# actionml/universal-recommender

Hardware: NVIDIA H100
Metric: CCO train events/sec to indicator model (higher is better)
Workload: dtype int32+f64

## Files before the change

universal_recommender_b200/csrc/cco_api.cu:

```cuda
#include <cuda_runtime.h>
#include <dlfcn.h>
#include <stdarg.h>
#include <stdio.h>
#include <stdlib.h>
#include <string.h>

#include <algorithm>
#include <cmath>
#include <functional>
#include <cub/cub.cuh>
#include <nvtx3/nvToolsExt.h>
#include <condition_variable>
#include <mutex>
#include <string>
#include <thread>
#include <unordered_map>
#include <vector>

#include "../../include/cco_b200.h"
#include "cco_kernels.cuh"
#include "cco_sampler.cuh"
#include "cco_format.cuh"
#include "cco_strings.cuh"
#include "cco_json.cuh"
// ... 637 lines not shown
  }
  CK(cudaEventRecord(stage_ev[2], s));
  if (W > 1) {
    g_nccl.GroupStart();
    for (int i = 0; i < n_mats; ++i) {
      if (!gathered[i]) continue;
      int rc = g_nccl.AllGather(gathered[i] + (size_t)r * cap[i], gathered[i], (size_t)cap[i], kNcclInt32, c->comm, s);
      if (rc != 0) { g_nccl.GroupEnd(); return nccl_check(rc, "ncclAllGather(column blocks)"); }
    }
    CKR(nccl_check(g_nccl.GroupEnd(), "ncclGroupEnd(column blocks)"));
    for (int i = 0; i < n_mats; ++i) {
      if (!gathered[i]) continue;
      dim3 grid((unsigned)std::max(1, std::min(c->sm_count * 8 / W, 1024)), (unsigned)W);
      k_pack_blocks<<<grid, 256, 0, s>>>(W, S, U, cap[i], dm[i].rp, gathered[i], dm[i].col);
      c->launches++;
      ar.release(gathered[i]);
    }
  }
  CK(cudaEventRecord(stage_ev[3], s));
  CK(cudaGetLastError());
  return CCO_OK;
}


struct BinCfg {
  int group;
  int slots;
  int cap;
  int cbuf;
  int caux, keep_max, final_max;
  bool dense;
  bool bitmap;
  int bm_words;
  size_t region;
  size_t smem;
  int ctas_per_sm;
};

static int next_pow2(int x) {
  int p = 1;
  while (p < x) p <<= 1;
  return p;
}

template <int GROUP>
static int launch_rows_t(cco_ctx *c, const RowArgs &a, BinCfg &cfg, cudaStream_t st) {
  constexpr int CTA = GROUP == 32 ? 64 : GROUP;
  int occ = 1;
  void (*kern)(const RowArgs) = cfg.dense ? k_rows<GROUP, true> : k_rows<GROUP, false>;
  if constexpr (GROUP == 512 || GROUP == 256)
    if (cfg.bitmap) kern = k_rows<GROUP, false, true>;
  CK(cudaFuncSetAttribute(kern, cudaFuncAttributeMaxDynamicSharedMemorySize, (int)cfg.smem));
  CK(cudaOccupancyMaxActiveBlocksPerMultiprocessor(&occ, kern, CTA, cfg.smem));
  kern<<<c->sm_count * std::max(occ, 1) * 4, CTA, cfg.smem, st>>>(a);
  cfg.ctas_per_sm = occ;
  c->launches++;
  CK(cudaGetLastError());
  return CCO_OK;
}
static int launch_rows(cco_ctx *c, const RowArgs &a, BinCfg &cfg, cudaStream_t st) {
  switch (cfg.group) {
    case 1024: return launch_rows_t<1024>(c, a, cfg, st);
    case 512: return launch_rows_t<512>(c, a, cfg, st);
    case 256: return launch_rows_t<256>(c, a, cfg, st);
    case 128: return launch_rows_t<128>(c, a, cfg, st);
    case 32: return launch_rows_t<32>(c, a, cfg, st);
  }
  return set_error(CCO_E_INVALID_ARG, "internal: bad bin config");
}

static BinCfg make_cfg(cco_ctx *c, int group, int want_slots, int top_k, int n_cols_b) {
  BinCfg f;
  const int groups = group == 32 ? 2 : 1;
  f.group = group;
  f.final_max = next_pow2(top_k);
  f.cbuf = next_pow2(top_k + std::max(group, 128) + (group == 32 ? 64 : 0));
  if (group == 32 && top_k + 32 <= 96) f.cbuf = 128;
  f.keep_max = std::max(f.final_max, (f.cbuf - group) / 2);
  f.caux = group == 32 ? 0 : f.keep_max;
  size_t fixed = (size_t)(f.cbuf + f.caux) * 16 + 2 * 256 + 512 + 1024 + (size_t)(group / 32) * 256;
  size_t avail = (c->smem_optin - 1024) / groups;
  int max_slots = (int)((avail - fixed) / 4) & ~1023;
  f.slots = std::min(want_slots, max_slots);
  f.cap = f.slots / 2;
  f.dense = n_cols_b <= f.slots;
  f.bitmap = false;
  f.bm_words = 0;
  f.region = (fixed + (size_t)f.slots * 4 + 15) & ~(size_t)15;
  f.smem = f.region * groups;
  f.ctas_per_sm = 1;
  return f;
}

static bool use_bitmap(BinCfg &f, uint32_t max_w, int top_k, int n_cols_b) {
  if (f.dense || (f.group != 512 && f.group != 256)) return false;
  const long long seg = 32LL * (f.group / 32);
  const long long rep = (std::max<long long>(max_w, 64) + seg - 1) / seg * seg;
  const long long bm = ((long long)n_cols_b + 31) / 32;
  if (rep + bm + top_k > f.slots) return false;
  f.bitmap = true;
  f.slots = (int)rep;
  f.bm_words = (int)bm;
  return true;
}

static double llr_error_bound(long long n_users) {
  const double n = (double)n_users;
  return n > 1.0 ? std::ldexp(n * std::log(n), -47) : 0.0;
}
static bool cut_exact(long long n_users, int32_t max_marg_a, int32_t max_marg_b) {
  const double n = (double)n_users, r = (double)max_marg_a, c = (double)max_marg_b;
  if (r <= 0.0 || c <= 0.0) return true;
  double g = 2.0 / std::min(r * c, 0.5 * n);
  const double d = n - c - r + 1.0;
  if (d > 0.0) g = std::max(g, 2.0 * (1.0 / c - (r - 1.0) / d));
  return g > 2.0 * llr_error_bound(n_users);
}

struct IndicatorState {
  int mail_group = -1;
// ... 43 lines not shown
  CKR(ar.alloc(&rows_sorted, n_items_a + 1));
  CK(cudaMemsetAsync(work64 + n_items_a, 0, 8, ss));
  k_row_work<<<grid_for((long long)n_items_a * kSG, 256, c->sm_count), 256, 0, ss>>>(n_items_a, at_ptr, at_users, B.rp,
                                                                                  row_work, work64, ids, nullptr);
  c->launches++;
  CKR(exclusive_sum(c, ar, (const long long *)work64, work_prefix, (long long)n_items_a + 1, ss));
  if (world > 1) {
    CKR(ar.alloc(&d_pb, world + 1));
    k_partition_rows<<<1, ((world + 1 + 31) / 32) * 32, 0, ss>>>(work_prefix, n_items_a, world, d_pb);
    c->launches++;
  }
  k_mask_work<<<grid_for(n_items_a, 256, c->sm_count), 256, 0, ss>>>(n_items_a, row_work, d_pb, rank, masked);
  c->launches++;
  if (n_items_a > 0) {
    void *tmp;
    CKR(ar.alloc((char **)&tmp, sort_tb));
    CK(cub::DeviceRadixSort::SortPairsDescending(tmp, sort_tb, masked, sorted_work, ids, rows_sorted, n_items_a, 0, 32, ss));
    ar.release(tmp);
  }
  const int k_eff = emit_all ? 1 : prm.top_k;
  const bool warp_ok = k_eff + 32 <= 256;
  struct BinSpec { int group, slots; uint32_t max_w; };
  std::vector<BinSpec> spec = {{1024, 1 << 20, 0xffffffffu}, {1024, 1 << 20, 0xffffffffu}, {512, 16384, 8192u}, {256, 8192, 4096u}};
  if (warp_ok) {
    spec.push_back({128, 4096, 2048u});
    spec.push_back({32, 2048, 1024u});
    spec.push_back({32, 1024, 512u});
    spec.push_back({32, 512, 256u});
  } else {
    spec.push_back({128, 4096, 2048u});
  }
  const int kBins = (int)spec.size();
  std::vector<BinCfg> cfgs(kBins);
  for (int b = 0; b < kBins; ++b) cfgs[b] = make_cfg(c, spec[b].group, spec[b].slots, k_eff, n_cols_b);
  BinCfg &cfgL = cfgs[1];
  int key_bits = 1;
  while (((1LL << key_bits) - 1) <= (long long)n_cols_b) ++key_bits;
  int count_bits = 32 - key_bits;
  const long long k11_max = std::min<long long>(max_marg_a, max_marg_b);
  if (count_bits < 1 || k11_max >= (1LL << count_bits))
    return set_error(CCO_E_UNSUPPORTED,
                     "co-occurrence counts up to %lld over %d columns do not fit the packed 32-bit accumulator word "
                     "(key %d bits + count %d bits): lower maxItemsPerUser/maxEventsPerEventType for this event type "
                     "(\"Limits\" in include/cco_b200.h)", k11_max, n_cols_b, key_bits, count_bits);
  std::vector<uint32_t> h_thr(kBins);
  for (int b = 0; b < kBins; ++b) {
    const BinCfg &f = cfgs[std::min(b + 1, kBins - 1)];
    uint32_t lim = b + 1 < kBins ? spec[b + 1].max_w : 0u;
    if (b + 1 < kBins && !f.dense) lim = std::min<uint32_t>(lim, (uint32_t)f.cap);
    h_thr[b] = lim;
    if (b > 0) h_thr[b] = std::min(h_thr[b], h_thr[b - 1]);
  }
  const bool bitmap_ok = !emit_all && cut_exact(n_users, max_marg_a, max_marg_b) &&
                         2ull * (unsigned long long)std::max(max_marg_a, 0) * (unsigned long long)std::max(max_marg_b, 0) <
                             (unsigned long long)n_users;
  for (int b = 1; b < kBins && bitmap_ok; ++b) use_bitmap(cfgs[b], h_thr[b - 1], k_eff, n_cols_b);
  int32_t *d_bounds;
  CKR(ar.alloc(&d_bounds, kBins + 3));
  BinThresholds bt;
  memset(&bt, 0, sizeof bt);
  for (int b = 0; b < kBins; ++b) bt.t[b] = h_thr[b];
  k_bin_bounds<<<1, 32, 0, ss>>>(n_items_a, sorted_work, kBins, bt, d_bounds);
  c->launches++;
  int32_t *key_of_col, *first_key_of_cb, *order_id0, *order_id1;
  uint32_t *order_cb0, *order_cb1;
  const int32_t n_order = std::max<int32_t>(n_cols_b, 1);
  CKR(ar.alloc(&key_of_col, n_order));
// ... 66 lines not shown
  a.self = self ? 1 : 0;
  a.top_k = k_eff;
  a.has_min_llr = prm.has_min_llr;
  a.min_llr = prm.min_llr;
  a.cut_ok = cut_exact(n_users, max_marg_a, max_marg_b) ? 1 : 0;
  a.llr_eps2 = 2.0 * llr_error_bound(n_users);
  a.flags = flags;
  a.count_bits = count_bits;
  a.out_stride = stride;
  a.out_col = o_col;
  a.out_llr = o_llr;
  a.out_cnt = o_cnt;
  a.out_len = o_len;
  a.stat_distinct = d_distinct;
  a.stat_evaluated = d_distinct + 1;
  a.err_flag = d_err;
  a.emit_all = emit_all ? 1 : 0;
  if (ev_begin) CK(cudaEventRecord(ev_begin, s));
  if (n_items_a > 0) {
    CK(cudaEventRecord(c->bin_ev[8], s));
    for (int b = 0; b < kBins; ++b) {
      if (b == 0 && cfgL.dense) continue;
      RowArgs ab = a;
      ab.bin = b;
      ab.slots = cfgs[b].slots;
      ab.cap = cfgs[b].cap;
      ab.tsize_x16 = 32;
      ab.cbuf = cfgs[b].cbuf;
      ab.caux = cfgs[b].caux;
      ab.keep_max = cfgs[b].keep_max;
      ab.final_max = cfgs[b].final_max;
      ab.group_smem_bytes = (int32_t)cfgs[b].region;
      ab.bm_words = cfgs[b].bm_words;
      CK(cudaStreamWaitEvent(c->bin_stream[b], c->bin_ev[8], 0));
      CKR(launch_rows(c, ab, cfgs[b], c->bin_stream[b]));
      CK(cudaEventRecord(c->bin_ev[b], c->bin_stream[b]));
      CK(cudaStreamWaitEvent(s, c->bin_ev[b], 0));
    }
  }
  if (ev_end) CK(cudaEventRecord(ev_end, s));
  long long *len64, *rec_d;
  CKR(ar.alloc(&len64, n_items_a + 1));
  CKR(ar.alloc(&st->out_ptr, n_items_a + 1));
  CKR(ar.alloc(&rec_d, 8));
  k_len_to_i64<<<grid_for((long long)n_items_a + 1, 256, c->sm_count), 256, 0, s>>>(n_items_a, o_len, d_pb, rank, len64);
  c->launches++;
  CKR(exclusive_sum(c, ar, len64, st->out_ptr, (long long)n_items_a + 1));
  CKR(ar.alloc(&st->p_col, cells));
  if (!(flags & CCO_FLAG_RESULT_NO_COUNT) || emit_all) CKR(ar.alloc(&st->p_cnt, cells));
  if (!emit_all && !(flags & CCO_FLAG_RESULT_NO_LLR)) CKR(ar.alloc(&st->p_llr, cells));
  if (n_items_a > 0) {
    k_compact_rows<<<grid_for((long long)n_items_a * 32, 256, c->sm_count), 256, 0, s>>>(n_items_a, stride, st->out_ptr, o_col, o_llr,
                                                                                      o_cnt, st->p_col, st->p_llr, st->p_cnt);
    c->launches++;
  }
  k_indicator_record<<<1, 32, 0, s>>>(n_items_a, d_pb, rank, st->out_ptr, work_prefix, d_distinct, d_err, rec_d);
  c->launches++;
  CKR(mail_fetch(c, st->rec, rec_d, sizeof(long long) * 7));
  CKR(mail_close(c, &st->mail_group));
  if (!st->packed) CK(cudaEventCreateWithFlags(&st->packed, cudaEventDisableTiming));
  CK(cudaEventRecord(st->packed, s));
  CK(cudaGetLastError());
  for (void *p : {(void *)o_col, (void *)o_cnt, (void *)o_llr, (void *)len64})
    if (p) ar.release(p);
  return CCO_OK;
}
// ... 4743 lines not shown
  CK(cudaMemcpyAsync(score, d_score, sizeof(double) * (size_t)n_items, cudaMemcpyDeviceToHost, s));
  CK(cudaMemcpyAsync(present, d_present, (size_t)n_items, cudaMemcpyDeviceToHost, s));
  CK(cudaStreamSynchronize(s));
  CK(cudaGetLastError());
  return CCO_OK;
}

void cco_free(void *p) { free(p); }

int cco_debug_llr(cco_ctx_t *c, int64_t n, const int64_t *k11, const int64_t *k12, const int64_t *k21, const int64_t *k22,
                  uint32_t flags, double *out) {
  if (!c || n < 0 || (n > 0 && (!k11 || !k12 || !k21 || !k22 || !out))) return set_error(CCO_E_INVALID_ARG, "bad argument");
  if (n == 0) return CCO_OK;
  for (int64_t i = 0; i < n; ++i)
    if (k11[i] < 0 || k12[i] < 0 || k21[i] < 0 || k22[i] < 0)
      return set_error(CCO_E_INVALID_ARG, "negative count at %lld (Preconditions.checkArgument in LogLikelihood)", (long long)i);
  CK(cudaSetDevice(c->device));
  Arena ar(c->stream);
  long long *d[4];
  double *dout;
  const int64_t *h[4] = {k11, k12, k21, k22};
  for (int j = 0; j < 4; ++j) {
    CKR(ar.alloc(&d[j], n));
    CK(cudaMemcpyAsync(d[j], h[j], sizeof(int64_t) * (size_t)n, cudaMemcpyHostToDevice, c->stream));
  }
  CKR(ar.alloc(&dout, n));
  k_debug_llr<<<(unsigned)((n + 255) / 256), 256, 0, c->stream>>>(n, d[0], d[1], d[2], d[3], flags, dout);
  CK(cudaMemcpyAsync(out, dout, sizeof(double) * (size_t)n, cudaMemcpyDeviceToHost, c->stream));
  CK(cudaStreamSynchronize(c->stream));
  CK(cudaGetLastError());
  return CCO_OK;
}

int cco_debug_rank_text(cco_ctx_t *c, int64_t n, const int64_t *v, int32_t scale, int64_t *offsets, char *bytes) {
  if (!c || n < 0 || !offsets || (n > 0 && (!v || !bytes))) return set_error(CCO_E_INVALID_ARG, "bad argument");
  if (scale != 0 && scale != 15) return set_error(CCO_E_INVALID_ARG, "scale %d is neither 0 nor 15", scale);
  for (int64_t i = 0; i < n; ++i)
    if (scale == 0 ? (v[i] <= -(1LL << 53) || v[i] >= (1LL << 53)) : (v[i] < 0 || v[i] >= 1000000000000000LL))
      return set_error(CCO_E_INVALID_ARG, "value %lld at %lld is outside the range of scale %d", (long long)v[i], (long long)i, scale);
  offsets[0] = 0;
  if (n == 0) return CCO_OK;
  CK(cudaSetDevice(c->device));
  cudaStream_t s = c->stream;
  Arena ar(s);
  long long *d_v;
  unsigned char *d_slot;
  int32_t *d_len;
  CKR(ar.alloc(&d_v, n));
  CKR(ar.alloc(&d_slot, 32 * n));
  CKR(ar.alloc(&d_len, n));
  CK(cudaMemcpyAsync(d_v, v, sizeof(int64_t) * (size_t)n, cudaMemcpyHostToDevice, s));
  k_debug_rank_text<<<grid_for(n, 256, c->sm_count), 256, 0, s>>>(n, d_v, scale, d_slot, d_len);
  std::vector<unsigned char> slot((size_t)32 * n);
  std::vector<int32_t> len((size_t)n);
  CK(cudaMemcpyAsync(slot.data(), d_slot, slot.size(), cudaMemcpyDeviceToHost, s));
  CK(cudaMemcpyAsync(len.data(), d_len, sizeof(int32_t) * (size_t)n, cudaMemcpyDeviceToHost, s));
  CK(cudaStreamSynchronize(s));
  CK(cudaGetLastError());
  for (int64_t i = 0; i < n; ++i) {
    if (len[i] < 1 || len[i] > 32) return set_error(CCO_E_CUDA, "text %lld has length %d", (long long)i, len[i]);
    memcpy(bytes + offsets[i], slot.data() + 32 * (size_t)i, (size_t)len[i]);
    offsets[i + 1] = offsets[i] + len[i];
  }
  return CCO_OK;
}

// ... 773 lines not shown
```

universal_recommender_b200/csrc/cco_kernels.cuh:

```cuda
#pragma once

#include <cuda_runtime.h>
#include <stdint.h>

namespace cco {

struct RowArgs {
  const uint32_t *at_ptr;
  const int32_t *at_users;
  const uint32_t *b_ptr;
  const int32_t *b_col;
  const int32_t *marg_a;
  const int32_t *marg_b;
  const int32_t *key_of_col;
  const int32_t *first_key_of_cb;
  int32_t key_shift;
  const uint2 *ext;
  int32_t max_marg_b;
  const int32_t *rows_sorted;
  const uint32_t *row_work;
  const int32_t *bin_bounds;
  int32_t bin;
  int32_t n_cols_b;
  long long n_users;
  int32_t self;
  int32_t top_k;
  int32_t has_min_llr;
  double min_llr;
  int32_t cut_ok;
  double llr_eps2;
  uint32_t flags;
  int32_t count_bits;
  int32_t slots;
  int32_t cap;
  int32_t tsize_x16;
  int32_t cbuf;
  int32_t caux;
  int32_t keep_max;
  int32_t final_max;
  int32_t group_smem_bytes;
  const struct ColTerm *col_terms;
  int32_t out_stride;
  int32_t *out_col;
  double *out_llr;
  int32_t *out_cnt;
  int32_t *out_len;
  unsigned long long *stat_distinct;
  unsigned long long *stat_evaluated;
  int *err_flag;
  int32_t emit_all;
  int32_t bm_words;
};

constexpr uint32_t kEmpty = 0xffffffffu;

__device__ __forceinline__ uint64_t mix64(uint64_t z) {
  z ^= z >> 30;
  z *= 0xbf58476d1ce4e5b9ULL;
  z ^= z >> 27;
  z *= 0x94d049bb133111ebULL;
  z ^= z >> 31;
  return z;
}
__device__ __forceinline__ double sample_u01(int32_t seed, uint32_t u, uint32_t j) {
  uint64_t x = mix64(((uint64_t)(uint32_t)seed << 32) | (uint64_t)u);
  uint64_t h = mix64(x + (uint64_t)j * 0x9e3779b97f4a7c15ULL);
  return __dmul_rn((double)(h >> 11), 0x1.0p-53);
}
__device__ __forceinline__ uint32_t hash32(uint32_t x) {
  x ^= x >> 16;
  x *= 0x7feb352dU;
  x ^= x >> 15;
  x *= 0x846ca68bU;
  x ^= x >> 16;
  return x;
}

__device__ __forceinline__ double xlogx(long long x) {
  return x == 0 ? 0.0 : __dmul_rn((double)x, log((double)x));
}
__device__ __forceinline__ double xlogx_u32(uint32_t x) {
  return x == 0 ? 0.0 : __dmul_rn((double)x, log((double)x));
}
__device__ __forceinline__ double entropy2(long long a, long long b, bool varargs) {
// ... 263 lines not shown
    t.col = col_of_key[i];
    t.pad[0] = t.pad[1] = 0;
    out[i] = t;
  }
}

__global__ void k_col_order_init(int32_t n_cols, const int32_t *__restrict__ marg, uint32_t *__restrict__ cb_out,
                                 int32_t *__restrict__ id_out) {
  for (int i = blockIdx.x * blockDim.x + threadIdx.x; i < n_cols; i += gridDim.x * blockDim.x) {
    cb_out[i] = (uint32_t)marg[i];
    id_out[i] = i;
  }
}
__global__ void k_col_order(int32_t n_cols, int32_t max_cb, const uint32_t *__restrict__ marg_key, const int32_t *__restrict__ col_of_key,
                            int32_t *__restrict__ key_of_col, int32_t *__restrict__ first_key_of_cb) {
  for (int k = blockIdx.x * blockDim.x + threadIdx.x; k < n_cols; k += gridDim.x * blockDim.x) {
    key_of_col[col_of_key[k]] = k;
    const int32_t cb = (int32_t)marg_key[k], lo = k == 0 ? 0 : (int32_t)marg_key[k - 1] + 1;
    for (int32_t c = lo; c <= cb; ++c) first_key_of_cb[c] = k;
    if (k == n_cols - 1)
      for (int32_t c = cb + 1; c <= max_cb + 1; ++c) first_key_of_cb[c] = n_cols;
  }
}
__global__ void k_relabel_cols(const uint32_t *__restrict__ end, const int32_t *__restrict__ key_of_col, int32_t *__restrict__ col) {
  const long long n = *end;
  for (long long q = blockIdx.x * (long long)blockDim.x + threadIdx.x; q < n; q += (long long)gridDim.x * blockDim.x)
    col[q] = key_of_col[col[q]];
}

__device__ __forceinline__ bool cand_better(const uint4 &p, const uint4 &q) {
  return p.y > q.y || (p.y == q.y && (p.x > q.x || (p.x == q.x && p.z < q.z)));
}

template <int GROUP>
__device__ __forceinline__ void group_sync() {
  if (GROUP == 32) __syncwarp(); else __syncthreads();
}

template <int GROUP>
__device__ void sort_candidates(uint4 *tk, int n, int gtid) {
  int n2 = 1;
  while (n2 < n) n2 <<= 1;
  for (int i = n + gtid; i < n2; i += GROUP) tk[i] = make_uint4(0u, 0u, 0xffffffffu, 0u);
  group_sync<GROUP>();
  for (int k2 = 2; k2 <= n2; k2 <<= 1) {
    for (int j = k2 >> 1; j > 0; j >>= 1) {
      for (int t = gtid; t < (n2 >> 1); t += GROUP) {
        const int i = ((t & ~(j - 1)) << 1) | (t & (j - 1));
        const int p = i | j;
        const bool up = (i & k2) == 0;
        const uint4 ei = tk[i], ep = tk[p];
        const bool swap = up ? cand_better(ep, ei) : cand_better(ei, ep);
        if (swap) { tk[i] = ep; tk[p] = ei; }
      }
      group_sync<GROUP>();
    }
  }
}

__device__ __forceinline__ uint32_t cand_word(const uint4 &e, int wi) { return wi == 0 ? e.y : (wi == 1 ? e.x : ~e.z); }

template <int GROUP>
__device__ int reduce_candidates(uint4 *tk, uint4 *aux, int n, int k, int M, int *hist, int *ctrl, int gtid) {
  volatile int *vc = ctrl;
  uint32_t pre0 = 0u, pre1 = 0u, pre2 = 0u;
  int nb = 0, above = 0, kept = n;
// ... 149 lines not shown
#pragma unroll
    for (int h = 0; h < 2; ++h) {
      const uint32_t p = p0 + h * 32 + lane;
      int j = 0;
#pragma unroll
      for (int st = 16; st > 0; st >>= 1) {
        const int c = j + st;
        const uint32_t v = __shfl_sync(0xffffffffu, off, c);
        if (v <= p) j = c;
      }
      const uint32_t sj = __shfl_sync(0xffffffffu, s, j), oj = __shfl_sync(0xffffffffu, off, j);
      act[h] = p < p_hi;
      bb[h] = act[h] ? (uint32_t)a.b_col[sj + (p - oj)] : 0u;
    }
    if (BITMAP) {
      uint32_t old[2];
#pragma unroll
      for (int h = 0; h < 2; ++h) old[h] = act[h] ? atomicOr(&seen[bb[h] >> 5], 1u << (bb[h] & 31u)) : 0u;
#pragma unroll
      for (int h = 0; h < 2; ++h)
        if (act[h] && ((old[h] >> (bb[h] & 31u)) & 1u)) accumulate<GROUP, false>(table, tsize, bb[h], cbits, 1u, 0u, a.err_flag);
    } else {
#pragma unroll
      for (int h = 0; h < 2; ++h)
        if (act[h]) accumulate<GROUP, DENSE>(table, tsize, bb[h], cbits, n_pass, pass, a.err_flag);
    }
  }
}

template <int GROUP>
struct RowsMinBlocks {
  static constexpr int value = GROUP == 512 ? 2 : GROUP == 256 ? 4 : GROUP == 128 ? 8 : GROUP == 32 ? 12 : 1;
};

template <int GROUP, bool DENSE, bool BITMAP = false>
__global__ void __launch_bounds__(GROUP == 32 ? 64 : GROUP, RowsMinBlocks<GROUP>::value) k_rows(const RowArgs a) {
  static_assert(!BITMAP || (GROUP > 32 && !DENSE), "bitmap rows are CTA-owned rows of a hashed bin");
  const int GROUPS = GROUP == 32 ? (int)(blockDim.x >> 5) : 1;
  constexpr int NW = GROUP / 32;
  extern __shared__ __align__(16) unsigned char smem_raw[];
  const int tid = threadIdx.x, lane = tid & 31;
  const int gid = tid / GROUP, gtid = tid % GROUP, gw = gtid >> 5;
  unsigned char *base = smem_raw + (size_t)gid * a.group_smem_bytes;
  uint4 *tk = reinterpret_cast<uint4 *>(base);
  uint4 *aux = tk + a.cbuf;
  double *x12tab = reinterpret_cast<double *>(aux + a.caux);
  double *x11tab = x12tab + 32;
  int *ctrl = reinterpret_cast<int *>(x11tab + 32);
  int *hist = ctrl + 128;
  uint32_t *wqueue = reinterpret_cast<uint32_t *>(hist + 256);
  uint32_t *h1 = reinterpret_cast<uint32_t *>(hist);
  uint32_t *table = wqueue + NW * 64;
  uint32_t *seen = table + a.slots;
  uint32_t *singles = seen + a.bm_words;
  volatile int *vctrl = ctrl;

  const int row_begin = a.bin_bounds[a.bin], row_end = a.bin_bounds[a.bin + 1];
  const bool varargs = (a.flags & CCO_FLAG_ENTROPY_VARARGS) != 0;
  const int cbits = a.count_bits;
  const uint32_t cmask = (1u << cbits) - 1u;
  const int prune_limit = a.cbuf - GROUP;
  const long long N = a.n_users;
  const double xN = xlogx(N);
  unsigned long long distinct_local = 0, evaluated_local = 0;
  if (gtid < 32) x11tab[gtid] = xlogx((long long)gtid);

  for (int ri = row_begin + blockIdx.x * GROUPS + gid; ri < row_end; ri += gridDim.x * GROUPS) {
    const int item = a.rows_sorted[ri];
    const uint32_t u_begin = a.at_ptr[item], u_end = a.at_ptr[item + 1];
    const long long ra = a.marg_a[item];
    const int diag = a.self ? a.key_of_col[item] : -1;
    const bool keyed = 2ull * (unsigned long long)ra * (unsigned long long)a.max_marg_b < (unsigned long long)N;
    uint32_t n_pass = 1, tsize = (uint32_t)a.n_cols_b;
    if (!DENSE) {
      const uint32_t w = a.row_work[item];
      const uint32_t dcells = BITMAP ? w / 2u : w;
      const uint32_t dbound = dcells < (uint32_t)a.n_cols_b ? dcells : (uint32_t)a.n_cols_b;
      n_pass = BITMAP ? 1u : (dbound + (uint32_t)a.cap - 1u) / (uint32_t)a.cap;
      if (n_pass == 0) n_pass = 1;
      tsize = n_pass > 1 ? (uint32_t)a.slots
                         : (uint32_t)min((unsigned long long)a.slots,
                                         max(((unsigned long long)dbound * (unsigned long long)a.tsize_x16) >> 4, 64ull));
      tsize = min((uint32_t)a.slots, (tsize + 32u * NW - 1u) / (32u * NW) * (32u * NW));
    }
    group_sync<GROUP>();
    if (gtid < 32) {
      const long long v = (gtid < kX12N) ? ra - gtid : N - ra;
      x12tab[gtid] = v >= 0 ? xlogx(v) : 0.0;
    }
    if (gtid == 0) { ctrl[0] = 0; ctrl[1] = 0; }
    if (gtid < 16) ctrl[40 + gtid] = 0x7fffffff;
    int emitted = 0;

    for (uint32_t pass = 0; pass < n_pass; ++pass) {
      for (uint32_t i = gtid; i < tsize; i += GROUP) table[i] = DENSE ? 0u : kEmpty;
      if (BITMAP)
        for (int i = gtid; i < a.bm_words; i += GROUP) seen[i] = 0u;
      group_sync<GROUP>();
// ... 34 lines not shown
            if (lane >= d) incl += v;
          }
          if (lane == 31) wsum[gw] = (int)incl;
          __syncthreads();
          uint32_t wpre = lane < NW ? (uint32_t)wsum[lane] : 0u;
#pragma unroll
          for (int d = 1; d < NW; d <<= 1) {
            const uint32_t v = __shfl_up_sync(0xffffffffu, wpre, d);
            if (lane >= d) wpre += v;
          }
          const uint32_t T = __shfl_sync(0xffffffffu, wpre, NW - 1);
          const uint32_t before = gw == 0 ? 0u : __shfl_sync(0xffffffffu, wpre, gw - 1);
          wofs[gtid] = make_uint2(s, before + incl - len);
          __syncthreads();
          const uint32_t p_lo = (uint32_t)((unsigned long long)T * gw / NW);
          const uint32_t p_hi = (uint32_t)((unsigned long long)T * (gw + 1) / NW);
          if (p_lo < p_hi) {
            uint32_t lo = 0, hi = nwin - 1;
            while (lo < hi) {
              const uint32_t mid = (lo + hi + 1) >> 1;
              if (wofs[mid].y <= p_lo) lo = mid; else hi = mid - 1;
            }
            for (uint32_t j0 = lo, p = p_lo; p < p_hi; j0 += 32) {
              const uint2 e = j0 + lane < nwin ? wofs[j0 + lane] : make_uint2(0u, 0xffffffffu);
              const uint32_t wend = min(p_hi, j0 + 32 < nwin ? wofs[j0 + 32].y : T);
              count_window<GROUP, DENSE, BITMAP>(a, table, seen, tsize, cbits, n_pass, pass, e.y, e.x, p, wend, lane);
              p = wend;
            }
          }
          __syncthreads();
        }
      }
      group_sync<GROUP>();
      const uint32_t seg = (((tsize + NW - 1) / NW) + 31u) & ~31u;
      const uint32_t seg_lo = min((uint32_t)gw * seg, tsize), seg_hi = min(seg_lo + seg, tsize);
      uint32_t n_mine = 0;
      for (uint32_t pos = seg_lo; pos < seg_hi; pos += 32) {
        const uint32_t idx = pos + lane;
        uint32_t w = DENSE ? 0u : kEmpty;
        if (idx < seg_hi) w = table[idx];
        const bool valid = DENSE ? (w != 0u) : (w != kEmpty);
        const uint32_t word = DENSE ? ((idx << cbits) | w) : w;
        const unsigned m = __ballot_sync(0xffffffffu, valid);
        __syncwarp();
        if (valid) {
          table[seg_lo + n_mine + __popc(m & ((1u << lane) - 1u))] = BITMAP ? word + 1u : word;
          if (BITMAP) atomicAnd(&seen[(word >> cbits) >> 5], ~(1u << ((word >> cbits) & 31u)));
        }
        n_mine += __popc(m);
        __syncwarp();
      }
      if (lane == 0) distinct_local += n_mine;
      uint32_t n_list = n_mine;
      const uint32_t *singles_mine = singles;
      if (BITMAP) {
        group_sync<GROUP>();
        if (gtid == 0 && diag >= 0) {
          const uint32_t bit = 1u << ((uint32_t)diag & 31u);
          if (seen[diag >> 5] & bit) {
            seen[diag >> 5] &= ~bit;
            ++distinct_local;
          }
        }
        group_sync<GROUP>();
        const uint32_t nbw = (uint32_t)a.bm_words, per = (nbw + GROUP - 1u) / GROUP;
        const uint32_t w_lo = min((uint32_t)gtid * per, nbw), w_hi = min(w_lo + per, nbw);
        uint32_t cnt = 0;
        for (uint32_t i = w_lo; i < w_hi; ++i) cnt += __popc(seen[i]);
        distinct_local += cnt;
        uint32_t incl = cnt;
#pragma unroll
        for (int d = 1; d < 32; d <<= 1) {
          const uint32_t v = __shfl_up_sync(0xffffffffu, incl, d);
          if (lane >= d) incl += v;
        }
        int *wsum = hist;
        if (lane == 31) wsum[gw] = (int)incl;
        __syncthreads();
        uint32_t wpre = lane < NW ? (uint32_t)wsum[lane] : 0u;
#pragma unroll
        for (int d = 1; d < NW; d <<= 1) {
          const uint32_t v = __shfl_up_sync(0xffffffffu, wpre, d);
          if (lane >= d) wpre += v;
        }
// ... 33 lines not shown
        uint32_t prefix = 0, need = (uint32_t)a.top_k;
        while (true) {
          for (int i = gtid; i < kCutBins / 2; i += GROUP) h1[i] = 0u;
          group_sync<GROUP>();
          for (uint32_t q0 = 0; q0 < n_mine; q0 += 32) {
            const uint32_t q = q0 + lane;
            if (q < n_mine) {
              const uint32_t word = table[seg_lo + q];
              const uint32_t b = word >> cbits;
              if ((word & cmask) == 1u && (int)b != diag) {
                uint32_t bin = kCutBins;
                if (keyed) {
                  if (((unsigned long long)(b ^ prefix) >> hi_sh) == 0) bin = (b >> sh) & (kCutBins - 1);
                } else {
                  const uint32_t cb = (uint32_t)a.marg_b[b];
                  if (cb < (uint32_t)kCutBins && 2ull * (unsigned long long)ra * cb < (unsigned long long)N) bin = cb;
                }
                if (bin < (uint32_t)kCutBins) atomicAdd(&h1[bin >> 1], 1u << (16u * (bin & 1u)));
              }
            }
          }
          group_sync<GROUP>();
          if (gtid < 32) cut_find(h1, need, lane, ctrl);
          group_sync<GROUP>();
          const int found = vctrl[9];
          if (!keyed || found == 0x7fffffff) { cut1 = found; break; }
          prefix |= (uint32_t)found << sh;
          need -= (uint32_t)vctrl[10];
          if (sh == 0) { cut1 = (int)prefix; break; }
          hi_sh = sh;
          sh = sh > 9 ? sh - 9 : 0;
        }
      }
      const double x_ra = x12tab[0], x_nra = x12tab[kX12N];
      const double row_e = varargs ? __dsub_rn(xN, __dadd_rn(__dadd_rn(0.0, x_ra), x_nra))
                                   : __dsub_rn(__dsub_rn(xN, x_ra), x_nra);
      uint32_t *wq = wqueue + gw * 64;
      uint32_t pos = 0;
      int qn = 0;
      while (true) {
        while (qn < 32 && pos < n_list) {
          const uint32_t q = pos + lane;
          bool surv = false;
          uint32_t word = 0;
          if (q < n_list) {
            word = (!BITMAP || q < n_mine) ? table[seg_lo + q] : singles_mine[q - n_mine];
            const uint32_t b = word >> cbits, k11 = word & cmask;
            if ((int)b != diag) {
              if (keyed) {
                surv = !(k11 <= (uint32_t)kDomLevels && (int)b >= vctrl[40 + k11]);
                if (k11 == 1u && (int)b > cut1) surv = false;
              } else {
                const long long cb = a.marg_b[b];
                const bool pos_side = (unsigned long long)ra * (unsigned long long)cb < (unsigned long long)k11 * (unsigned long long)N;
                surv = !(pos_side && k11 <= (uint32_t)kDomLevels && (int)cb >= vctrl[40 + k11]);
                if (k11 == 1u && (int)cb > cut1 && 2ull * (unsigned long long)ra * (unsigned long long)cb < (unsigned long long)N)
                  surv = false;
              }
            }
          }
          const unsigned m = __ballot_sync(0xffffffffu, surv);
          if (surv) wq[qn + __popc(m & ((1u << lane) - 1u))] = word;
          qn += __popc(m);
          pos += 32;
          __syncwarp();
        }
        const int take = qn < 32 ? qn : 32;
        bool pass_ok = false;
        uint4 e = make_uint4(0u, 0u, 0u, 0u);
        if (lane < take) {
          const uint32_t word = wq[qn - take + lane];
          const uint32_t b = word >> cbits, k11 = word & cmask;
          const ColTerm ct = a.col_terms[b];
          const long long cb = ct.cb;
          const bool pos_side = (unsigned long long)ra * (unsigned long long)cb < (unsigned long long)k11 * (unsigned long long)N;
          const uint32_t kf = k11 < (uint32_t)kDomLevels ? k11 : (uint32_t)kDomLevels;
          ++evaluated_local;
          const long long k21 = cb - k11, k22 = N - ra - cb + k11;
          const double x11 = k11 < 32 ? x11tab[k11] : xlogx_u32(k11);
          const double x12 = k11 < kX12N ? x12tab[k11] : xlogx_u32((uint32_t)(ra - k11));
          const double x21 = k11 == 1 ? ct.x_cbm1 : xlogx_u32((uint32_t)k21), x22 = xlogx_u32((uint32_t)k22);
          double mat_e;
          if (varargs)
            mat_e = __dsub_rn(xN, __dadd_rn(__dadd_rn(__dadd_rn(__dadd_rn(0.0, x11), x12), x21), x22));
          else
            mat_e = __dsub_rn(__dsub_rn(__dsub_rn(__dsub_rn(xN, x11), x12), x21), x22);
          const double sre = __dadd_rn(row_e, ct.col_e);
          const double v = (sre < mat_e) ? 0.0 : __dmul_rn(2.0, __dsub_rn(sre, mat_e));
          const bool min_ok = !a.has_min_llr || v >= a.min_llr;
          pass_ok = v > 0.0 && min_ok;
          const double vm = __dadd_rn(v, a.llr_eps2);
          bool strict_fail = v > 0.0 && !min_ok && vm < a.min_llr;
          const unsigned long long key = (unsigned long long)__double_as_longlong(v);
          e = make_uint4((uint32_t)key, (uint32_t)(key >> 32), (uint32_t)ct.col, k11);
          if (pass_ok && vctrl[1]) {
            const uint4 thr = make_uint4((uint32_t)vctrl[4], (uint32_t)vctrl[5], (uint32_t)vctrl[6], (uint32_t)vctrl[7]);
            pass_ok = !cand_better(thr, e);
            strict_fail = vm < __hiloint2double((int)thr.y, (int)thr.x);
          }
          if (strict_fail && pos_side) {
            const int f = keyed ? a.first_key_of_cb[cb] : (int)cb;
            for (uint32_t kk = kf; kk >= 1 && f < vctrl[40 + kk]; --kk) atomicMin(&ctrl[40 + kk], f);
          }
        }
        qn -= take;
        const unsigned m = __ballot_sync(0xffffffffu, pass_ok);
        int basepos_round = 0;
        if (m) {
          int basepos = 0;
          if (lane == 0) basepos = atomicAdd(&ctrl[0], __popc(m));
          basepos = __shfl_sync(0xffffffffu, basepos, 0);
          if (pass_ok) tk[basepos + __popc(m & ((1u << lane) - 1u))] = e;
          basepos_round = basepos;
        }
        const bool more = qn > 0 || pos < n_list;
        int mine = 0;
        if (m) mine = basepos_round + __popc(m);
        bool any_more, need_prune;
        if (GROUP == 32) {
          __syncwarp();
          any_more = more;
          need_prune = mine > prune_limit;
        } else {
          any_more = __syncthreads_or(more ? 1 : 0) != 0;
          need_prune = __syncthreads_or(mine > prune_limit ? 1 : 0) != 0;
        }
        if (need_prune) {
          const int n = vctrl[0];
          if (GROUP > 32 && n <= 512) {
            if (gw == 0) reduce_candidates<32>(tk, aux, n, a.top_k, a.keep_max, hist, ctrl, lane);
            group_sync<GROUP>();
          } else {
            reduce_candidates<GROUP>(tk, aux, n, a.top_k, a.keep_max, hist, ctrl, gtid);
          }
        }
        if (!any_more) break;
      }
      group_sync<GROUP>();
    }
    if (a.emit_all) {
      if (gtid == 0) a.out_len[item] = emitted;
    } else {
      int n = vctrl[0];
      if (n > 0) {
        if (GROUP > 32 && n <= 512) {
          if (gw == 0) {
            int m = n;
            if (m > a.final_max) m = reduce_candidates<32>(tk, aux, m, a.top_k, a.final_max, hist, ctrl, lane);
            sort_candidates<32>(tk, m, lane);
            if (lane == 0) ctrl[0] = m;
          }
          group_sync<GROUP>();
          n = vctrl[0];
        } else {
          if (n > a.final_max) n = reduce_candidates<GROUP>(tk, aux, n, a.top_k, a.final_max, hist, ctrl, gtid);
          sort_candidates<GROUP>(tk, n, gtid);
        }
        const int keep = n < a.top_k ? n : a.top_k;
        for (int i = gtid; i < keep; i += GROUP) {
          const size_t o = (size_t)item * a.out_stride + i;
          const uint4 e = tk[i];
          a.out_col[o] = (int32_t)e.z;
          a.out_llr[o] = __longlong_as_double((long long)(((unsigned long long)e.y << 32) | e.x));
          a.out_cnt[o] = (int32_t)e.w;
        }
        if (gtid == 0) a.out_len[item] = keep;
      } else if (gtid == 0) {
        a.out_len[item] = 0;
      }
    }
  }
  for (int o = 16; o > 0; o >>= 1) distinct_local += __shfl_xor_sync(0xffffffffu, distinct_local, o);
  if (lane == 0 && distinct_local) atomicAdd(a.stat_distinct, distinct_local);
  for (int o = 16; o > 0; o >>= 1) evaluated_local += __shfl_xor_sync(0xffffffffu, evaluated_local, o);
  if (lane == 0 && evaluated_local) atomicAdd(a.stat_evaluated, evaluated_local);
}

__global__ void k_compact_rows(int32_t n_items, int32_t stride, const long long *__restrict__ out_ptr,
                               const int32_t *__restrict__ col, const double *__restrict__ llr, const int32_t *__restrict__ cnt,
                               int32_t *__restrict__ p_col, double *__restrict__ p_llr, int32_t *__restrict__ p_cnt) {
  int warp = (blockIdx.x * blockDim.x + threadIdx.x) >> 5, lane = threadIdx.x & 31;
  int nwarps = (gridDim.x * blockDim.x) >> 5;
  for (int item = warp; item < n_items; item += nwarps) {
    const long long o = out_ptr[item];
    const int n = (int)(out_ptr[item + 1] - o);
    size_t src = (size_t)item * stride;
    for (int i = lane; i < n; i += 32) {
      p_col[o + i] = col[src + i];
      if (p_llr) p_llr[o + i] = llr[src + i];
      if (p_cnt) p_cnt[o + i] = cnt[src + i];
    }
  }
}

__global__ void k_expand_keys(long long n_rows, const long long *__restrict__ rp, const int32_t *__restrict__ col,
                              unsigned long long *__restrict__ keys) {
  const int lane = threadIdx.x % kSG;
  long long row = (blockIdx.x * (long long)blockDim.x + threadIdx.x) / kSG;
  const long long stride = (long long)gridDim.x * blockDim.x / kSG;
  const long long q_base = rp[0];
  for (; row < n_rows; row += stride) {
    long long s = rp[row], e = rp[row + 1];
    for (long long q = s + lane; q < e; q += kSG) keys[q - q_base] = ((unsigned long long)row << 32) | (uint32_t)col[q];
  }
// ... 148 lines not shown
```

Measured before the change: 4.381 billion.

## Keep warp-group top-k candidates in registers via bitonic shuffle merges

New measurement: 4.528 billion, median of 6. +3.4%, better.

```diff
diff --git a/universal_recommender_b200/csrc/cco_api.cu b/universal_recommender_b200/csrc/cco_api.cu
--- a/universal_recommender_b200/csrc/cco_api.cu
+++ b/universal_recommender_b200/csrc/cco_api.cu
@@ -693,6 +693,7 @@
   bool dense;
   bool bitmap;
   int bm_words;
+  bool reg_select;
   size_t region;
   size_t smem;
   int ctas_per_sm;
@@ -730,7 +731,7 @@
   return set_error(CCO_E_INVALID_ARG, "internal: bad bin config");
 }
 
-static BinCfg make_cfg(cco_ctx *c, int group, int want_slots, int top_k, int n_cols_b) {
+static BinCfg make_cfg(cco_ctx *c, int group, int want_slots, int top_k, int n_cols_b, bool emit_all) {
   BinCfg f;
   const int groups = group == 32 ? 2 : 1;
   f.group = group;
@@ -747,6 +748,11 @@
   f.dense = n_cols_b <= f.slots;
   f.bitmap = false;
   f.bm_words = 0;
+  f.reg_select = group == 32 && !f.dense && top_k <= 64 && !emit_all;
+  if (f.reg_select) {
+    fixed -= (size_t)f.cbuf * 16;
+    f.cbuf = 0;
+  }
   f.region = (fixed + (size_t)f.slots * 4 + 15) & ~(size_t)15;
   f.smem = f.region * groups;
   f.ctas_per_sm = 1;
@@ -856,7 +862,7 @@
   }
   const int kBins = (int)spec.size();
   std::vector<BinCfg> cfgs(kBins);
-  for (int b = 0; b < kBins; ++b) cfgs[b] = make_cfg(c, spec[b].group, spec[b].slots, k_eff, n_cols_b);
+  for (int b = 0; b < kBins; ++b) cfgs[b] = make_cfg(c, spec[b].group, spec[b].slots, k_eff, n_cols_b, emit_all);
   BinCfg &cfgL = cfgs[1];
   int key_bits = 1;
   while (((1LL << key_bits) - 1) <= (long long)n_cols_b) ++key_bits;
@@ -989,6 +995,7 @@
       ab.final_max = cfgs[b].final_max;
       ab.group_smem_bytes = (int32_t)cfgs[b].region;
       ab.bm_words = cfgs[b].bm_words;
+      ab.reg_select = cfgs[b].reg_select ? 1 : 0;
       CK(cudaStreamWaitEvent(c->bin_stream[b], c->bin_ev[8], 0));
       CKR(launch_rows(c, ab, cfgs[b], c->bin_stream[b]));
       CK(cudaEventRecord(c->bin_ev[b], c->bin_stream[b]));
@@ -5798,6 +5805,18 @@
   return CCO_OK;
 }
 
+#ifdef CCO_ROW_PHASES
+extern "C" int cco_debug_row_phases(cco_ctx_t *c, unsigned long long *out) {
+  if (!c || !out) return set_error(CCO_E_INVALID_ARG, "bad argument");
+  CK(cudaSetDevice(c->device));
+  CK(cudaDeviceSynchronize());
+  CK(cudaMemcpyFromSymbol(out, g_row_phases, sizeof g_row_phases));
+  static const unsigned long long zero[kPhaseBins][kPhaseFields] = {};
+  CK(cudaMemcpyToSymbol(g_row_phases, zero, sizeof zero));
+  return CCO_OK;
+}
+#endif
+
 int cco_debug_rank_text(cco_ctx_t *c, int64_t n, const int64_t *v, int32_t scale, int64_t *offsets, char *bytes) {
   if (!c || n < 0 || !offsets || (n > 0 && (!v || !bytes))) return set_error(CCO_E_INVALID_ARG, "bad argument");
   if (scale != 0 && scale != 15) return set_error(CCO_E_INVALID_ARG, "scale %d is neither 0 nor 15", scale);
diff --git a/universal_recommender_b200/csrc/cco_kernels.cuh b/universal_recommender_b200/csrc/cco_kernels.cuh
--- a/universal_recommender_b200/csrc/cco_kernels.cuh
+++ b/universal_recommender_b200/csrc/cco_kernels.cuh
@@ -50,6 +50,7 @@
   int *err_flag;
   int32_t emit_all;
   int32_t bm_words;
+  int32_t reg_select;
 };
 
 constexpr uint32_t kEmpty = 0xffffffffu;
@@ -379,6 +380,41 @@
   return p.y > q.y || (p.y == q.y && (p.x > q.x || (p.x == q.x && p.z < q.z)));
 }
 
+struct RegCand {
+  unsigned long long k;
+  uint32_t p;
+};
+__device__ __forceinline__ RegCand no_cand() { return RegCand{0ull, 0xffffffffu}; }
+__device__ __forceinline__ bool rc_better(const RegCand &x, const RegCand &y) { return x.k > y.k || (x.k == y.k && x.p < y.p); }
+__device__ __forceinline__ RegCand rc_shfl(const RegCand &x, int src) {
+  return RegCand{__shfl_sync(0xffffffffu, x.k, src), __shfl_sync(0xffffffffu, x.p, src)};
+}
+__device__ __forceinline__ RegCand rc_step(const RegCand &x, int j, bool keep_better) {
+  const RegCand o{__shfl_xor_sync(0xffffffffu, x.k, j), __shfl_xor_sync(0xffffffffu, x.p, j)};
+  return rc_better(o, x) == keep_better ? o : x;
+}
+__device__ __forceinline__ RegCand rc_bitonic_merge(RegCand x, int lane) {
+#pragma unroll
+  for (int j = 16; j > 0; j >>= 1) x = rc_step(x, j, (lane & j) == 0);
+  return x;
+}
+__device__ __forceinline__ void rc_merge(RegCand &h0, RegCand &h1, RegCand b, int n, bool two, int lane) {
+  const bool asc = n > 0;
+#pragma unroll
+  for (int k = 2; k <= 32; k <<= 1)
+#pragma unroll
+    for (int j = k >> 1; j > 0; j >>= 1) b = rc_step(b, j, ((lane & j) == 0) == (((lane & k) == 0) != asc));
+  if (n == 0) {
+    h0 = b;
+    return;
+  }
+  if (two && n > 32) b = rc_shfl(rc_bitonic_merge(rc_better(h1, b) ? h1 : b, lane), 31 - lane);
+  const bool hb = rc_better(h0, b);
+  const RegCand hi = hb ? h0 : b, lo = hb ? b : h0;
+  h0 = rc_bitonic_merge(hi, lane);
+  h1 = rc_bitonic_merge(lo, lane);
+}
+
 template <int GROUP>
 __device__ __forceinline__ void group_sync() {
   if (GROUP == 32) __syncwarp(); else __syncthreads();
@@ -594,6 +630,26 @@
 struct RowsMinBlocks {
   static constexpr int value = GROUP == 512 ? 2 : GROUP == 256 ? 4 : GROUP == 128 ? 8 : GROUP == 32 ? 12 : 1;
 };
+
+constexpr int kPhaseBins = 8, kPhaseFields = 16;
+#ifdef CCO_ROW_PHASES
+__device__ unsigned long long g_row_phases[kPhaseBins][kPhaseFields];
+#define CCO_PHASE(i)                             \
+  do {                                           \
+    if (GROUP == 32) {                           \
+      const long long t_ = clock64();            \
+      ph[i] += (unsigned long long)(t_ - ph_t);  \
+      ph_t = t_;                                 \
+    }                                            \
+  } while (0)
+#define CCO_PHASE_ADD(i, v) \
+  do {                      \
+    if (GROUP == 32) ph[i] += (unsigned long long)(v); \
+  } while (0)
+#else
+#define CCO_PHASE(i) do {} while (0)
+#define CCO_PHASE_ADD(i, v) do {} while (0)
+#endif
 
 template <int GROUP, bool DENSE, bool BITMAP = false>
 __global__ void __launch_bounds__(GROUP == 32 ? 64 : GROUP, RowsMinBlocks<GROUP>::value) k_rows(const RowArgs a) {
@@ -616,6 +672,7 @@
   uint32_t *seen = table + a.slots;
   uint32_t *singles = seen + a.bm_words;
   volatile int *vctrl = ctrl;
+  const bool reg = GROUP == 32 && !DENSE && !BITMAP && a.reg_select != 0;
 
   const int row_begin = a.bin_bounds[a.bin], row_end = a.bin_bounds[a.bin + 1];
   const bool varargs = (a.flags & CCO_FLAG_ENTROPY_VARARGS) != 0;
@@ -626,6 +683,10 @@
   const double xN = xlogx(N);
   unsigned long long distinct_local = 0, evaluated_local = 0;
   if (gtid < 32) x11tab[gtid] = xlogx((long long)gtid);
+#ifdef CCO_ROW_PHASES
+  unsigned long long ph[kPhaseFields] = {};
+  long long ph_t = clock64();
+#endif
 
   for (int ri = row_begin + blockIdx.x * GROUPS + gid; ri < row_end; ri += gridDim.x * GROUPS) {
     const int item = a.rows_sorted[ri];
@@ -726,6 +787,7 @@
         }
       }
       group_sync<GROUP>();
+      CCO_PHASE(1);
       const uint32_t seg = (((tsize + NW - 1) / NW) + 31u) & ~31u;
       const uint32_t seg_lo = min((uint32_t)gw * seg, tsize), seg_hi = min(seg_lo + seg, tsize);
       uint32_t n_mine = 0;
@@ -744,6 +806,7 @@
         n_mine += __popc(m);
         __syncwarp();
       }
+      CCO_PHASE(2);
       if (lane == 0) distinct_local += n_mine;
       uint32_t n_list = n_mine;
       const uint32_t *singles_mine = singles;
@@ -843,12 +906,15 @@
           sh = sh > 9 ? sh - 9 : 0;
         }
       }
+      CCO_PHASE(3);
       const double x_ra = x12tab[0], x_nra = x12tab[kX12N];
       const double row_e = varargs ? __dsub_rn(xN, __dadd_rn(__dadd_rn(0.0, x_ra), x_nra))
                                    : __dsub_rn(__dsub_rn(xN, x_ra), x_nra);
       uint32_t *wq = wqueue + gw * 64;
       uint32_t pos = 0;
       int qn = 0;
+      RegCand rc0 = no_cand(), rc1 = no_cand();
+      int rseen = 0;
       while (true) {
         while (qn < 32 && pos < n_list) {
           const uint32_t q = pos + lane;
@@ -879,6 +945,8 @@
         const int take = qn < 32 ? qn : 32;
         bool pass_ok = false;
         uint4 e = make_uint4(0u, 0u, 0u, 0u);
+        RegCand re = no_cand();
+        const RegCand rthr = reg && rseen >= a.top_k ? rc_shfl(a.top_k > 32 ? rc1 : rc0, (a.top_k - 1) & 31) : no_cand();
         if (lane < take) {
           const uint32_t word = wq[qn - take + lane];
           const uint32_t b = word >> cbits, k11 = word & cmask;
@@ -903,11 +971,19 @@
           const double vm = __dadd_rn(v, a.llr_eps2);
           bool strict_fail = v > 0.0 && !min_ok && vm < a.min_llr;
           const unsigned long long key = (unsigned long long)__double_as_longlong(v);
-          e = make_uint4((uint32_t)key, (uint32_t)(key >> 32), (uint32_t)ct.col, k11);
-          if (pass_ok && vctrl[1]) {
-            const uint4 thr = make_uint4((uint32_t)vctrl[4], (uint32_t)vctrl[5], (uint32_t)vctrl[6], (uint32_t)vctrl[7]);
-            pass_ok = !cand_better(thr, e);
-            strict_fail = vm < __hiloint2double((int)thr.y, (int)thr.x);
+          if (reg) {
+            re = RegCand{key, ((uint32_t)ct.col << cbits) | k11};
+            if (pass_ok && rseen >= a.top_k) {
+              pass_ok = rc_better(re, rthr);
+              strict_fail = vm < __longlong_as_double((long long)rthr.k);
+            }
+          } else {
+            e = make_uint4((uint32_t)key, (uint32_t)(key >> 32), (uint32_t)ct.col, k11);
+            if (pass_ok && vctrl[1]) {
+              const uint4 thr = make_uint4((uint32_t)vctrl[4], (uint32_t)vctrl[5], (uint32_t)vctrl[6], (uint32_t)vctrl[7]);
+              pass_ok = !cand_better(thr, e);
+              strict_fail = vm < __hiloint2double((int)thr.y, (int)thr.x);
+            }
           }
           if (strict_fail && pos_side) {
             const int f = keyed ? a.first_key_of_cb[cb] : (int)cb;
@@ -916,6 +992,17 @@
         }
         qn -= take;
         const unsigned m = __ballot_sync(0xffffffffu, pass_ok);
+        if (reg) {
+          if (m) {
+            CCO_PHASE(4);
+            rc_merge(rc0, rc1, pass_ok ? re : no_cand(), rseen, a.top_k > 32, lane);
+            rseen += __popc(m);
+            CCO_PHASE(5);
+            CCO_PHASE_ADD(8, __popc(m));
+          }
+          if (qn > 0 || pos < n_list) continue;
+          break;
+        }
         int basepos_round = 0;
         if (m) {
           int basepos = 0;
@@ -923,6 +1010,7 @@
           basepos = __shfl_sync(0xffffffffu, basepos, 0);
           if (pass_ok) tk[basepos + __popc(m & ((1u << lane) - 1u))] = e;
           basepos_round = basepos;
+          CCO_PHASE_ADD(8, __popc(m));
         }
         const bool more = qn > 0 || pos < n_list;
         int mine = 0;
@@ -937,6 +1025,8 @@
           need_prune = __syncthreads_or(mine > prune_limit ? 1 : 0) != 0;
         }
         if (need_prune) {
+          CCO_PHASE(4);
+          CCO_PHASE_ADD(7, 1);
           const int n = vctrl[0];
           if (GROUP > 32 && n <= 512) {
             if (gw == 0) reduce_candidates<32>(tk, aux, n, a.top_k, a.keep_max, hist, ctrl, lane);
@@ -944,14 +1034,31 @@
           } else {
             reduce_candidates<GROUP>(tk, aux, n, a.top_k, a.keep_max, hist, ctrl, gtid);
           }
+          CCO_PHASE(5);
         }
         if (!any_more) break;
       }
       group_sync<GROUP>();
+      CCO_PHASE(4);
+      if (reg) {
+        const int keep = rseen < a.top_k ? rseen : a.top_k;
+        const size_t o = (size_t)item * a.out_stride + lane;
+        if (lane < keep) {
+          a.out_col[o] = (int32_t)(rc0.p >> cbits);
+          a.out_llr[o] = __longlong_as_double((long long)rc0.k);
+          a.out_cnt[o] = (int32_t)(rc0.p & cmask);
+        }
+        if (32 + lane < keep) {
+          a.out_col[o + 32] = (int32_t)(rc1.p >> cbits);
+          a.out_llr[o + 32] = __longlong_as_double((long long)rc1.k);
+          a.out_cnt[o + 32] = (int32_t)(rc1.p & cmask);
+        }
+        if (lane == 0) a.out_len[item] = keep;
+      }
     }
     if (a.emit_all) {
       if (gtid == 0) a.out_len[item] = emitted;
-    } else {
+    } else if (!reg) {
       int n = vctrl[0];
       if (n > 0) {
         if (GROUP > 32 && n <= 512) {
@@ -980,7 +1087,13 @@
         a.out_len[item] = 0;
       }
     }
-  }
+    CCO_PHASE(6);
+    CCO_PHASE_ADD(0, 1);
+  }
+#ifdef CCO_ROW_PHASES
+  if (GROUP == 32 && lane == 0 && a.bin < kPhaseBins)
+    for (int i = 0; i < kPhaseFields; ++i) atomicAdd(&g_row_phases[a.bin][i], ph[i]);
+#endif
   for (int o = 16; o > 0; o >>= 1) distinct_local += __shfl_xor_sync(0xffffffffu, distinct_local, o);
   if (lane == 0 && distinct_local) atomicAdd(a.stat_distinct, distinct_local);
   for (int o = 16; o > 0; o >>= 1) evaluated_local += __shfl_xor_sync(0xffffffffu, evaluated_local, o);
```
